# hangxu0304/DeepReduce

Hardware: NVIDIA H100
Metric: ResNet-50 images/sec (whole job, device-timed, max over ranks) (higher is better)
Workload: dtype bf16

## Files before the change

### deepreduce_b200/models/resnet.py

```python
from __future__ import annotations

import torch.nn as nn
import torch.nn.functional as F

from .fused_bn import bn_add_relu, bn_bn_add_relu, bn_relu, bn_relu_maxpool


class _BasicCifar(nn.Module):
    def __init__(self, inp, out, stride):
        super().__init__()
        self.conv1 = nn.Conv2d(inp, out, 3, stride, 1, bias=False)
        self.bn1 = nn.BatchNorm2d(out)
        self.conv2 = nn.Conv2d(out, out, 3, 1, 1, bias=False)
        self.bn2 = nn.BatchNorm2d(out)
        self.pad = None
        if stride != 1 or inp != out:
            self.pad = (out - inp, stride)

    def forward(self, x):
        y = F.relu(self.bn1(self.conv1(x)))
        y = self.bn2(self.conv2(y))
        if self.pad is not None:
            extra, s = self.pad
            x = F.pad(x[:, :, ::s, ::s], (0, 0, 0, 0, extra // 2, extra - extra // 2))
        return F.relu(x + y)


class ResNetCifar(nn.Module):
    def __init__(self, n: int = 3, num_classes: int = 10):
        super().__init__()
        self.conv1 = nn.Conv2d(3, 16, 3, 1, 1, bias=False)
        self.bn1 = nn.BatchNorm2d(16)
        layers, inp = [], 16
        for out, stride in ((16, 1), (32, 2), (64, 2)):
            for i in range(n):
                layers.append(_BasicCifar(inp, out, stride if i == 0 else 1))
                inp = out
        self.layers = nn.Sequential(*layers)
        self.fc = nn.Linear(64, num_classes)

    def forward(self, x):
        x = F.relu(self.bn1(self.conv1(x)))
        x = self.layers(x)
        x = F.adaptive_avg_pool2d(x, 1).flatten(1)
        return self.fc(x)


def resnet20(num_classes: int = 10) -> ResNetCifar:
    return ResNetCifar(3, num_classes)


class _Bottleneck(nn.Module):
    expansion = 4

    def __init__(self, inp, width, stride, downsample):
        super().__init__()
        out = width * self.expansion
        self.conv1 = nn.Conv2d(inp, width, 1, bias=False)
        self.bn1 = nn.BatchNorm2d(width)
        self.conv2 = nn.Conv2d(width, width, 3, stride, 1, bias=False)
        self.bn2 = nn.BatchNorm2d(width)
        self.conv3 = nn.Conv2d(width, out, 1, bias=False)
        self.bn3 = nn.BatchNorm2d(out)
        self.downsample = None
        if downsample:
            self.downsample = nn.Sequential(nn.Conv2d(inp, out, 1, stride, bias=False), nn.BatchNorm2d(out))

    def forward(self, x, skip=None, fork=False):
        skip = x if skip is None else skip
        xd = None if self.downsample is None else self.downsample[0](skip)
        y = bn_relu(self.conv1(x), self.bn1)
        y = bn_relu(self.conv2(y), self.bn2)
        y = self.conv3(y)
        if xd is None:
            return bn_add_relu(y, self.bn3, skip, fork=fork)
        o = bn_bn_add_relu(y, self.bn3, xd, self.downsample[1])
        return (o, None) if fork else o


class ResNet(nn.Module):
    def __init__(self, blocks=(3, 4, 6, 3), num_classes: int = 1000):
        super().__init__()
        self.conv1 = nn.Conv2d(3, 64, 7, 2, 3, bias=False)
        self.bn1 = nn.BatchNorm2d(64)
        self.maxpool = nn.MaxPool2d(3, 2, 1)
        stages, inp = [], 64
        for i, (n, width) in enumerate(zip(blocks, (64, 128, 256, 512))):
            for j in range(n):
                stride = 2 if (j == 0 and i > 0) else 1
                stages.append(_Bottleneck(inp, width, stride, downsample=(j == 0)))
                inp = width * 4
        self.layers = nn.Sequential(*stages)
        self.fc = nn.Linear(inp, num_classes)
        for m in self.modules():
            if isinstance(m, nn.Conv2d):
                nn.init.kaiming_normal_(m.weight, mode="fan_out", nonlinearity="relu")

    def forward(self, x):
        x, skip = bn_relu_maxpool(self.conv1(x), self.bn1, self.maxpool), None
        for blk in self.layers:
            x, skip = blk(x, skip, fork=True)
        x = F.adaptive_avg_pool2d(x, 1).flatten(1)
        return self.fc(x)


def resnet50(num_classes: int = 1000) -> ResNet:
    return ResNet((3, 4, 6, 3), num_classes)
```

### deepreduce_b200/ops/csrc/bn.cu

```cuda
#include <cuda_bf16.h>

#include <algorithm>

#include "common.cuh"
#include "ops.h"

namespace dr {

namespace {

constexpr int kVec = 8;
constexpr int kApplyThreads = 256;
constexpr int kReduceThreads = 128;

struct ChanParams {
  float m[kVec], inv[kVec], w[kVec], b[kVec];
};

__device__ __forceinline__ void load8(const float* __restrict__ p, float* d) {
  const float4 a = __ldg(reinterpret_cast<const float4*>(p));
  const float4 b = __ldg(reinterpret_cast<const float4*>(p) + 1);
  d[0] = a.x; d[1] = a.y; d[2] = a.z; d[3] = a.w;
  d[4] = b.x; d[5] = b.y; d[6] = b.z; d[7] = b.w;
}

__device__ __forceinline__ void load_params(const BnParams& p, int c, ChanParams& o) {
  load8(p.mean + c, o.m);
  load8(p.invstd + c, o.inv);
  load8(p.weight + c, o.w);
  load8(p.bias + c, o.b);
}

__device__ __forceinline__ float bn_elem(float x, float m, float inv, float w, float b) {
  return __fmaf_rn(__fmul_rn(w, __fsub_rn(x, m)), inv, b);
}

__device__ __forceinline__ __nv_bfloat16 relu_bf16(__nv_bfloat16 v) {
  return __bfloat162float(v) <= 0.f ? __float2bfloat16_rn(0.f) : v;
}

__device__ __forceinline__ uint4 add_bf16x8(const uint4& a, const uint4& b) {
  uint4 s;
  const __nv_bfloat16* ha = reinterpret_cast<const __nv_bfloat16*>(&a);
  const __nv_bfloat16* hb = reinterpret_cast<const __nv_bfloat16*>(&b);
  __nv_bfloat16* hs = reinterpret_cast<__nv_bfloat16*>(&s);
#pragma unroll
  for (int i = 0; i < kVec; ++i) hs[i] = __float2bfloat16_rn(__fadd_rn(__bfloat162float(ha[i]), __bfloat162float(hb[i])));
  return s;
}

template <int kMode>
__global__ void __launch_bounds__(kApplyThreads) bn_apply_kernel(const __nv_bfloat16* __restrict__ x, BnParams px,
                                                                 const __nv_bfloat16* __restrict__ z, BnParams pz,
                                                                 __nv_bfloat16* __restrict__ out,
                                                                 uint8_t* __restrict__ mask, int64_t rows, int C) {
  const int groups = C / kVec;
  const int rows_per_cta = blockDim.x / groups;
  const int rsub = threadIdx.x / groups;
  if (rsub >= rows_per_cta) return;
  const int c = (threadIdx.x % groups) * kVec;
  ChanParams a;
  load_params(px, c, a);
  ChanParams d;
  if (kMode == 2) load_params(pz, c, d);
  const int64_t step = (int64_t)gridDim.x * rows_per_cta;
#pragma unroll 2
  for (int64_t r = (int64_t)blockIdx.x * rows_per_cta + rsub; r < rows; r += step) {
    const int64_t off = r * C + c;
    const uint4 vx = *reinterpret_cast<const uint4*>(x + off);
    uint4 vz = make_uint4(0, 0, 0, 0);
    if (kMode != 0) vz = *reinterpret_cast<const uint4*>(z + off);
    const __nv_bfloat16* hx = reinterpret_cast<const __nv_bfloat16*>(&vx);
    const __nv_bfloat16* hz = reinterpret_cast<const __nv_bfloat16*>(&vz);
    uint4 vo;
    __nv_bfloat16* ho = reinterpret_cast<__nv_bfloat16*>(&vo);
    unsigned bits = 0;
#pragma unroll
    for (int i = 0; i < kVec; ++i) {
      __nv_bfloat16 y = __float2bfloat16_rn(bn_elem(__bfloat162float(hx[i]), a.m[i], a.inv[i], a.w[i], a.b[i]));
      if (kMode != 0) {
        const __nv_bfloat16 s = kMode == 1 ? hz[i]
                                           : __float2bfloat16_rn(bn_elem(__bfloat162float(hz[i]), d.m[i], d.inv[i], d.w[i], d.b[i]));
        y = __float2bfloat16_rn(__fadd_rn(__bfloat162float(y), __bfloat162float(s)));
      }
      ho[i] = relu_bf16(y);
      bits |= (__bfloat162float(ho[i]) <= 0.f ? 0u : 1u) << i;
    }
    *reinterpret_cast<uint4*>(out + off) = vo;
    mask[r * groups + c / kVec] = (uint8_t)bits;
  }
}


__global__ void __launch_bounds__(kApplyThreads) bn_apply_pool_kernel(const __nv_bfloat16* __restrict__ x, BnParams px,
                                                                      __nv_bfloat16* __restrict__ out,
                                                                      uint8_t* __restrict__ codes, int64_t orows,
                                                                      PoolGeom pg, int C) {
  const int groups = C / kVec;
  const int rows_per_cta = blockDim.x / groups;
  const int rsub = threadIdx.x / groups;
  if (rsub >= rows_per_cta) return;
  const int c = (threadIdx.x % groups) * kVec;
  ChanParams a;
  load_params(px, c, a);
  const int64_t step = (int64_t)gridDim.x * rows_per_cta;
  for (int64_t r = (int64_t)blockIdx.x * rows_per_cta + rsub; r < orows; r += step) {
    const int ow = (int)(r % pg.Wo);
    const int64_t t = r / pg.Wo;
    const int oh = (int)(t % pg.Ho);
    const int64_t n = t / pg.Ho;
    const int h0 = 2 * oh - 1, w0 = 2 * ow - 1;
    uint4 v[9];
#pragma unroll
    for (int k = 0; k < 9; ++k) {
      const int ih = h0 + k / 3, iw = w0 + k % 3;
      v[k] = ih >= 0 && ih < pg.H && iw >= 0 && iw < pg.W
                 ? *reinterpret_cast<const uint4*>(x + ((n * pg.H + ih) * pg.W + iw) * C + c)
                 : uint4{};
    }
    __nv_bfloat16 best[kVec];
    unsigned slot[kVec];
#pragma unroll
    for (int i = 0; i < kVec; ++i) {
      best[i] = __float2bfloat16_rn(-INFINITY);
      slot[i] = 0;
    }
#pragma unroll
    for (int k = 0; k < 9; ++k) {
      const int ih = h0 + k / 3, iw = w0 + k % 3;
      if (ih < 0 || ih >= pg.H || iw < 0 || iw >= pg.W) continue;
      const __nv_bfloat16* hx = reinterpret_cast<const __nv_bfloat16*>(&v[k]);
#pragma unroll
      for (int i = 0; i < kVec; ++i) {
        const __nv_bfloat16 y = relu_bf16(__float2bfloat16_rn(bn_elem(__bfloat162float(hx[i]), a.m[i], a.inv[i], a.w[i], a.b[i])));
        const float fy = __bfloat162float(y);
        if (fy > __bfloat162float(best[i]) || isnan(fy)) {
          best[i] = y;
          slot[i] = k;
        }
      }
    }
    uint4 vo;
    __nv_bfloat16* ho = reinterpret_cast<__nv_bfloat16*>(&vo);
    uint2 vc;
    uint8_t* hc = reinterpret_cast<uint8_t*>(&vc);
#pragma unroll
    for (int i = 0; i < kVec; ++i) {
      ho[i] = best[i];
      hc[i] = (uint8_t)(slot[i] | (__bfloat162float(best[i]) <= 0.f ? 0u : 0x80u));
    }
    *reinterpret_cast<uint4*>(out + r * C + c) = vo;
    *reinterpret_cast<uint2*>(codes + r * C + c) = vc;
  }
}

struct PoolGather {
  uint4 g[4];
  uint2 code[4];
  int off;
  int nh, nw;
  int sh, sw;
};

__device__ __forceinline__ void pool_gather_codes(PoolGather& q, const uint8_t* __restrict__ codes, const PoolGeom& pg,
                                                  int row, int C, int c, bool valid) {
  const int w = row % pg.W, t = row / pg.W, h = t % pg.H, n = t / pg.H;
  const int ph = h >> 1, pw = w >> 1;
  q.nh = valid ? min((h + 1) / 2 + 1, pg.Ho) - ph : 0;
  q.nw = valid ? min((w + 1) / 2 + 1, pg.Wo) - pw : 0;
  q.sh = h - 2 * ph + 1;
  q.sw = w - 2 * pw + 1;
  q.off = ((n * pg.Ho + ph) * pg.Wo + pw) * C + c;
#pragma unroll
  for (int k = 0; k < 4; ++k) {
    const int a = k >> 1, b = k & 1;
    q.code[k] = a < q.nh && b < q.nw ? *reinterpret_cast<const uint2*>(codes + q.off + (a * pg.Wo + b) * C) : uint2{};
  }
}

template <bool kTwo>
__device__ __forceinline__ void pool_gather_grads(PoolGather& q, const __nv_bfloat16* __restrict__ gp,
                                                  const __nv_bfloat16* __restrict__ gp2, const PoolGeom& pg, int C) {
#pragma unroll
  for (int k = 0; k < 4; ++k) {
    const int a = k >> 1, b = k & 1;
    const bool in = a < q.nh && b < q.nw;
    const int off = q.off + (a * pg.Wo + b) * C;
    q.g[k] = in ? *reinterpret_cast<const uint4*>(gp + off) : uint4{};
    if (kTwo && in) q.g[k] = add_bf16x8(q.g[k], *reinterpret_cast<const uint4*>(gp2 + off));
  }
}

__device__ __forceinline__ void pool_gather_resolve(const PoolGather& q, uint4& g, unsigned& bits) {
  __nv_bfloat16* hg = reinterpret_cast<__nv_bfloat16*>(&g);
  const bool single = q.nh == 1 && q.nw == 1;
  bits = 0;
#pragma unroll
  for (int i = 0; i < kVec; ++i) {
    float s = 0.f;
    __nv_bfloat16 one = __float2bfloat16_rn(0.f);
    unsigned bit = 0;
#pragma unroll
    for (int k = 0; k < 4; ++k) {
      const int a = k >> 1, b = k & 1;
      const unsigned code = (reinterpret_cast<const uint8_t*>(&q.code[k]))[i];
      if (a < q.nh && b < q.nw && (int)(code & 0x7fu) == (q.sh - 2 * a) * 3 + (q.sw - 2 * b)) {
        const __nv_bfloat16 v = (reinterpret_cast<const __nv_bfloat16*>(&q.g[k]))[i];
        s = __fadd_rn(s, __bfloat162float(v));
        one = v;
        bit = code >> 7;
      }
    }
    hg[i] = single ? one : __float2bfloat16_rn(s);
    bits |= bit << i;
  }
}

template <bool kTwo>
__global__ void __launch_bounds__(kApplyThreads) bn_pool_grad_kernel(const __nv_bfloat16* __restrict__ gp,
                                                                     const __nv_bfloat16* __restrict__ gp2,
                                                                     const uint8_t* __restrict__ codes,
                                                                     __nv_bfloat16* __restrict__ g, PoolGeom pg,
                                                                     int64_t rows, int C) {
  const int groups = C / kVec;
  const int rows_per_cta = blockDim.x / groups;
  const int rsub = threadIdx.x / groups;
  if (rsub >= rows_per_cta) return;
  const int c = (threadIdx.x % groups) * kVec;
  const int64_t step = (int64_t)gridDim.x * rows_per_cta;
#pragma unroll 2
  for (int64_t r = (int64_t)blockIdx.x * rows_per_cta + rsub; r < rows; r += step) {
    PoolGather q;
    pool_gather_codes(q, codes, pg, (int)r, C, c, true);
    pool_gather_grads<kTwo>(q, gp, gp2, pg, C);
    uint4 v;
    unsigned bits;
    pool_gather_resolve(q, v, bits);
    __nv_bfloat16* hv = reinterpret_cast<__nv_bfloat16*>(&v);
#pragma unroll
    for (int i = 0; i < kVec; ++i)
      if (!((bits >> i) & 1u)) hv[i] = __float2bfloat16_rn(0.f);
    *reinterpret_cast<uint4*>(g + r * C + c) = v;
  }
}

struct RowTree {
  int block_y, grid_y;
  __host__ __device__ int S() const { return block_y * grid_y; }
  __host__ __device__ int loops(int rows) const { return 1 + (rows - 1) / (S() * kLoads); }
  static constexpr int kLoads = 4;
};

constexpr int kStatsThreads = 256;

__device__ __forceinline__ void welford_update(float x, float inv, float valid, float& mean, float& m2n) {
  const float d0 = __fsub_rn(x, mean);
  mean = __fmaf_rn(d0, inv, mean);
  const float d1 = __fsub_rn(x, mean);
  m2n = __fmaf_rn(__fmul_rn(d0, d1), valid, m2n);
}

template <int kN, bool kFuseNew>
__device__ __forceinline__ void welford_merge(int& n, float* mean, float* m2n, int n_new, const float* mean_new,
                                              const float* m2n_new) {
  const float fn = (float)n, fn_new = (float)n_new;
  const float factor = __frcp_rn((float)max(1, n + n_new));
#pragma unroll
  for (int i = 0; i < kN; ++i) {
    const float d = __fsub_rn(mean[i], mean_new[i]);
    const float s = kFuseNew ? __fmaf_rn(mean_new[i], fn_new, __fmul_rn(mean[i], fn))
                             : __fmaf_rn(mean[i], fn, __fmul_rn(mean_new[i], fn_new));
    mean[i] = __fmul_rn(s, factor);
    const float u = __fmul_rn(__fmul_rn(__fmul_rn(d, d), fn_new), fn);
    m2n[i] = __fadd_rn(m2n[i], __fmaf_rn(u, factor, m2n_new[i]));
  }
  n += n_new;
}

template <int kN>
struct WelfordSlots {
  float* mean; float* m2n; int* count;
  __device__ WelfordSlots(float* sh, int slots)
      : mean(sh), m2n(sh + slots * kN), count(reinterpret_cast<int*>(sh + 2 * slots * kN)) {}
  __device__ void put(int s, int n, const float* m, const float* q) const {
#pragma unroll
    for (int i = 0; i < kN; ++i) { mean[s * kN + i] = m[i]; m2n[s * kN + i] = q[i]; }
    count[s] = n;
  }
  template <bool kFuseNew>
  __device__ void merge_from(int s, int& n, float* m, float* q) const {
    float mn[kN], qn[kN];
#pragma unroll
    for (int i = 0; i < kN; ++i) { mn[i] = mean[s * kN + i]; qn[i] = m2n[s * kN + i]; }
    welford_merge<kN, kFuseNew>(n, m, q, count[s], mn, qn);
  }
  static size_t bytes(int slots) { return (size_t)slots * (2 * kN * sizeof(float) + sizeof(int)); }
};

template <int kN>
__device__ __forceinline__ void welford_tree_over_y(const WelfordSlots<kN>& sl, bool part, int y, int block_y, int base,
                                                    int stride, int& n, float* mean, float* m2n) {
  for (int off = block_y / 2; off > 0; off >>= 1) {
    if (part && y < 2 * off) sl.put(base + y * stride, n, mean, m2n);
    __syncthreads();
    if (part && y < off) sl.template merge_from<false>(base + (y + off) * stride, n, mean, m2n);
    __syncthreads();
  }
}

struct StatsOut {
  float* mean; float* invstd; float* running_mean; float* running_var;
  float* st_mean; float* st_m2n; int* st_count;
  float momentum, bessel, eps;
};

__device__ __forceinline__ void stats_store(const StatsOut& o, int c, int n, float mean, float m2n) {
  const float var = __fdiv_rn(m2n, (float)n);
  const float keep = __fsub_rn(1.f, o.momentum);
  o.mean[c] = mean;
  o.invstd[c] = rsqrtf(__fadd_rn(var, o.eps));
  o.running_mean[c] = __fmaf_rn(mean, o.momentum, __fmul_rn(o.running_mean[c], keep));
  o.running_var[c] = __fmaf_rn(__fmul_rn(var, o.bessel), o.momentum, __fmul_rn(o.running_var[c], keep));
}

__global__ void __launch_bounds__(kStatsThreads) bn_stats_kernel(const __nv_bfloat16* __restrict__ x, StatsOut o,
                                                                 RowTree t, int rows, int C) {
  constexpr int L = RowTree::kLoads;
  constexpr int kAhead = 4;
  extern __shared__ float sh[];
  const int gpc = blockDim.x / (L * t.block_y);
  const int g = threadIdx.x % gpc, j = (threadIdx.x / gpc) % L, y = threadIdx.x / (gpc * L);
  const int group = blockIdx.x * gpc + g;
  const bool live = group * kVec < C;
  const int c = live ? group * kVec : 0;
  const int S = t.S();
  const int n_loops = t.loops(rows);
  const int r0 = blockIdx.y * t.block_y + y + j * S;
  const int rstep = L * S;
  float mean[kVec], m2n[kVec];
#pragma unroll
  for (int i = 0; i < kVec; ++i) mean[i] = m2n[i] = 0.f;
  int n = 0;
  auto load = [&](uint4* b, int i0) {
#pragma unroll
    for (int u = 0; u < kAhead; ++u) {
      const int r = r0 + (i0 + u) * rstep;
      b[u] = live && i0 + u < n_loops && r < rows ? *reinterpret_cast<const uint4*>(x + (size_t)r * C + c) : uint4{};
    }
  };
  uint4 cur[kAhead];
  load(cur, 0);
  for (int i0 = 0; i0 < n_loops; i0 += kAhead) {
    uint4 nxt[kAhead];
    load(nxt, i0 + kAhead);
#pragma unroll
    for (int u = 0; u < kAhead; ++u) {
      const int i = i0 + u;
      if (i >= n_loops) break;
      const bool valid = r0 + i * rstep < rows;
      const float inv = valid ? __frcp_rn((float)(i + 1)) : 0.f;
      const float fv = valid ? 1.f : 0.f;
      n += valid;
      const __nv_bfloat16* hx = reinterpret_cast<const __nv_bfloat16*>(&cur[u]);
#pragma unroll
      for (int k = 0; k < kVec; ++k) welford_update(__bfloat162float(hx[k]), inv, fv, mean[k], m2n[k]);
    }
#pragma unroll
    for (int u = 0; u < kAhead; ++u) cur[u] = nxt[u];
  }
  const WelfordSlots<kVec> sl(sh, blockDim.x);
  sl.put(threadIdx.x, n, mean, m2n);
  __syncthreads();
  if (j == 0) {
#pragma unroll
    for (int a = 1; a < L; ++a) sl.merge_from<true>(threadIdx.x + a * gpc, n, mean, m2n);
  }
  __syncthreads();
  welford_tree_over_y<kVec>(sl, j == 0, y, t.block_y, g, gpc * L, n, mean, m2n);
  if (j != 0 || y != 0 || !live) return;
  if (t.grid_y == 1) {
#pragma unroll
    for (int i = 0; i < kVec; ++i) stats_store(o, c + i, n, mean[i], m2n[i]);
    return;
  }
#pragma unroll
  for (int i = 0; i < kVec; ++i) {
    o.st_mean[(size_t)blockIdx.y * C + c + i] = mean[i];
    o.st_m2n[(size_t)blockIdx.y * C + c + i] = m2n[i];
  }
  if (group == 0) o.st_count[blockIdx.y] = n;
}

__global__ void bn_stats_finalize_kernel(StatsOut o, RowTree t, int C) {
  extern __shared__ float sh[];
  const int cols = blockDim.x / t.block_y;
  const int col = threadIdx.x % cols, y = threadIdx.x / cols;
  const int c = blockIdx.x * cols + col;
  int n = 0;
  float mean = 0.f, m2n = 0.f;
  if (c < C)
    for (int b = y; b < t.grid_y; b += t.block_y) {
      const float mb = o.st_mean[(size_t)b * C + c], qb = o.st_m2n[(size_t)b * C + c];
      welford_merge<1, false>(n, &mean, &m2n, o.st_count[b], &mb, &qb);
    }
  const WelfordSlots<1> sl(sh, blockDim.x);
  welford_tree_over_y<1>(sl, true, y, t.block_y, col, cols, n, &mean, &m2n);
  if (y == 0 && c < C) stats_store(o, c, n, mean, m2n);
}


template <int kN>
__device__ __forceinline__ void tree_over_y(float* v, float* sh, int y, int n, int col, int width) {
  for (int off = n / 2; off > 0; off >>= 1) {
#pragma unroll
    for (int i = 0; i < kN; ++i) sh[y * width + col + i] = v[i];
    __syncthreads();
    if (y < off) {
#pragma unroll
      for (int i = 0; i < kN; ++i) v[i] = __fadd_rn(v[i], sh[(y + off) * width + col + i]);
    }
    __syncthreads();
  }
}

struct BwdOut {
  float* sums;
  float* dw; float* db; float* dwz; float* dbz;
  float* staging;
};

__device__ __forceinline__ void bwd_store(const BwdOut& o, int k, int c, int C, float v, const float* invstd,
                                         const float* invstd_z) {
  o.sums[k * C + c] = v;
  if (k == 0) {
    o.db[c] = v;
    if (o.dbz) o.dbz[c] = v;
  } else if (k == 1) {
    o.dw[c] = __fmul_rn(v, invstd[c]);
  } else {
    o.dwz[c] = __fmul_rn(v, invstd_z[c]);
  }
}

__device__ __forceinline__ float masked(__nv_bfloat16 go, unsigned bit) { return bit ? __bfloat162float(go) : 0.f; }

template <int kMode, bool kTwo>
__global__ void __launch_bounds__(kReduceThreads) bn_bwd_reduce_kernel(const __nv_bfloat16* __restrict__ go,
                                                                       const __nv_bfloat16* __restrict__ go2,
                                                                       const uint8_t* __restrict__ mask,
                                                                       const __nv_bfloat16* __restrict__ x,
                                                                       const float* __restrict__ mean,
                                                                       const float* __restrict__ invstd,
                                                                       const __nv_bfloat16* __restrict__ z,
                                                                       const float* __restrict__ mean_z,
                                                                       const float* __restrict__ invstd_z,
                                                                       __nv_bfloat16* __restrict__ g_out, BwdOut o,
                                                                       RowTree t, int rows, int C) {
  constexpr int kSums = kMode == 2 ? 3 : 2;
  constexpr int L = RowTree::kLoads;
  extern __shared__ float sh[];
  const int gpc = blockDim.x / t.block_y;
  const int tg = threadIdx.x % gpc, y = threadIdx.x / gpc;
  const int group = blockIdx.x * gpc + tg;
  const bool live = group * kVec < C;
  const int c = live ? group * kVec : 0;
  const int S = t.S();
  float m[kVec], mz[kVec];
#pragma unroll
  for (int i = 0; i < kVec; ++i) {
    m[i] = mean[c + i];
    mz[i] = kMode == 2 ? mean_z[c + i] : 0.f;
  }
  float acc[kSums][L][kVec];
#pragma unroll
  for (int k = 0; k < kSums; ++k)
#pragma unroll
    for (int j = 0; j < L; ++j)
#pragma unroll
      for (int i = 0; i < kVec; ++i) acc[k][j][i] = 0.f;
  const int mgroups = C / kVec;
  int r = blockIdx.y * t.block_y + y;
  const int n_loops = t.loops(rows);
  constexpr bool kAhead = !(kTwo && kMode == 2);
  struct Batch {
    uint4 g[L], g2[L], x[L], z[L];
    unsigned m[L];
  };
  auto load = [&](Batch& b, int r0) {
#pragma unroll
    for (int j = 0; j < L; ++j) {
      const int rr = r0 + j * S;
      if (live && rr < rows) {
        const int off = rr * C + c;
        b.g[j] = *reinterpret_cast<const uint4*>(go + off);
        if (kTwo) b.g2[j] = *reinterpret_cast<const uint4*>(go2 + off);
        b.x[j] = *reinterpret_cast<const uint4*>(x + off);
        if (kMode == 2) b.z[j] = *reinterpret_cast<const uint4*>(z + off);
        b.m[j] = kMode == 3 ? 0u : mask[rr * mgroups + group];
      } else {
        b.g[j] = uint4{}; b.g2[j] = uint4{}; b.x[j] = uint4{}; b.z[j] = uint4{}; b.m[j] = 0;
      }
    }
  };
  Batch cur;
  if (kAhead) load(cur, r);
  for (int it = 0; it < n_loops; ++it) {
    if (!kAhead) load(cur, r);
    if (kTwo) {
#pragma unroll
      for (int j = 0; j < L; ++j) cur.g[j] = add_bf16x8(cur.g[j], cur.g2[j]);
    }
    Batch nxt;
    if (kAhead) load(nxt, r + L * S);
    const unsigned* mb = cur.m;
#pragma unroll
    for (int j = 0; j < L; ++j) {
      const __nv_bfloat16* hg = reinterpret_cast<const __nv_bfloat16*>(&cur.g[j]);
      const __nv_bfloat16* hx = reinterpret_cast<const __nv_bfloat16*>(&cur.x[j]);
      const __nv_bfloat16* hz = reinterpret_cast<const __nv_bfloat16*>(&cur.z[j]);
      uint4 vo;
      __nv_bfloat16* ho = reinterpret_cast<__nv_bfloat16*>(&vo);
#pragma unroll
      for (int i = 0; i < kVec; ++i) {
        const unsigned bit = (mb[j] >> i) & 1u;
        const float g = kMode == 3 ? __bfloat162float(hg[i]) : masked(hg[i], bit);
        if (kMode == 1) ho[i] = bit ? hg[i] : __float2bfloat16_rn(0.f);
        acc[0][j][i] = __fadd_rn(acc[0][j][i], g);
        acc[1][j][i] = __fmaf_rn(__fsub_rn(__bfloat162float(hx[i]), m[i]), g, acc[1][j][i]);
        if (kMode == 2) acc[2][j][i] = __fmaf_rn(__fsub_rn(__bfloat162float(hz[i]), mz[i]), g, acc[2][j][i]);
      }
      if (kMode == 1 && live && r + j * S < rows) *reinterpret_cast<uint4*>(g_out + (r + j * S) * C + c) = vo;
    }
    if (kAhead) cur = nxt;
    r += L * S;
  }
#pragma unroll
  for (int k = 0; k < kSums; ++k) {
#pragma unroll
    for (int i = 0; i < kVec; ++i)
#pragma unroll
      for (int j = 1; j < L; ++j) acc[k][0][i] = __fadd_rn(acc[k][0][i], acc[k][j][i]);
    tree_over_y<kVec>(acc[k][0], sh, y, t.block_y, tg * kVec, gpc * kVec);
  }
  if (y != 0 || !live) return;
#pragma unroll
  for (int k = 0; k < kSums; ++k)
#pragma unroll
    for (int i = 0; i < kVec; ++i) {
      if (t.grid_y > 1) o.staging[((size_t)k * t.grid_y + blockIdx.y) * C + c + i] = acc[k][0][i];
      else bwd_store(o, k, c + i, C, acc[k][0][i], invstd, invstd_z);
    }
}

__global__ void bn_bwd_finalize_kernel(BwdOut o, RowTree t, int n_sums, int C, const float* __restrict__ invstd,
                                       const float* __restrict__ invstd_z) {
  extern __shared__ float sh[];
  const int cols = blockDim.x / t.block_y;
  const int col = threadIdx.x % cols, y = threadIdx.x / cols;
  const int c = blockIdx.x * cols + col;
  for (int k = 0; k < n_sums; ++k) {
    float v = 0.f;
    if (c < C)
      for (int b = y; b < t.grid_y; b += t.block_y) v = __fadd_rn(v, o.staging[((size_t)k * t.grid_y + b) * C + c]);
    tree_over_y<1>(&v, sh, y, t.block_y, col, cols);
    if (y == 0 && c < C) bwd_store(o, k, c, C, v, invstd, invstd_z);
  }
}

struct ElemtChan {
  float m[kVec], f1[kVec], f2[kVec], sdy[kVec];
};

__device__ __forceinline__ void elemt_params(const float* mean, const float* invstd, const float* w, const float* sdy,
                                             const float* sxmu, float norm, int c, ElemtChan& p) {
  float inv[kVec], ww[kVec], sx[kVec];
  load8(mean + c, p.m);
  load8(invstd + c, inv);
  load8(w + c, ww);
  load8(sdy + c, p.sdy);
  load8(sxmu + c, sx);
#pragma unroll
  for (int i = 0; i < kVec; ++i) {
    p.f1[i] = __fmul_rn(__fmul_rn(__fmul_rn(inv[i], inv[i]), sx[i]), norm);
    p.f2[i] = __fmul_rn(ww[i], inv[i]);
  }
}

__device__ __forceinline__ __nv_bfloat16 elemt(float g, float x, const ElemtChan& p, int i, float norm) {
  const float a = __fmaf_rn(-p.sdy[i], norm, g);
  return __float2bfloat16_rn(__fmul_rn(__fmaf_rn(-p.f1[i], __fsub_rn(x, p.m[i]), a), p.f2[i]));
}

struct ElemtArgs {
  const float *mean, *invstd, *weight, *sums;
  const float *mean_z, *invstd_z, *weight_z;
};

template <int kMode, bool kTwo>
__global__ void __launch_bounds__(kApplyThreads) bn_bwd_elemt_kernel(const __nv_bfloat16* __restrict__ g_in,
                                                                     const __nv_bfloat16* __restrict__ g2_in,
                                                                     const uint8_t* __restrict__ mask,
                                                                     const __nv_bfloat16* __restrict__ x,
                                                                     const __nv_bfloat16* __restrict__ z, ElemtArgs a,
                                                                     __nv_bfloat16* __restrict__ dx,
                                                                     __nv_bfloat16* __restrict__ dz, float norm,
                                                                     int64_t rows, int C) {
  const int groups = C / kVec;
  const int rows_per_cta = blockDim.x / groups;
  const int rsub = threadIdx.x / groups;
  if (rsub >= rows_per_cta) return;
  const int c = (threadIdx.x % groups) * kVec;
  ElemtChan p;
  elemt_params(a.mean, a.invstd, a.weight, a.sums, a.sums + C, norm, c, p);
  ElemtChan q;
  if (kMode == 2) elemt_params(a.mean_z, a.invstd_z, a.weight_z, a.sums, a.sums + 2 * C, norm, c, q);
  const int64_t step = (int64_t)gridDim.x * rows_per_cta;
#pragma unroll 2
  for (int64_t r = (int64_t)blockIdx.x * rows_per_cta + rsub; r < rows; r += step) {
    const int64_t off = r * C + c;
    uint4 vg = *reinterpret_cast<const uint4*>(g_in + off);
    if (kTwo) vg = add_bf16x8(vg, *reinterpret_cast<const uint4*>(g2_in + off));
    const unsigned mb = kMode == 1 || kMode == 3 ? 0xffu : mask[r * groups + c / kVec];
    const uint4 vx = *reinterpret_cast<const uint4*>(x + off);
    uint4 vz = make_uint4(0, 0, 0, 0);
    if (kMode == 2) vz = *reinterpret_cast<const uint4*>(z + off);
    const __nv_bfloat16* hg = reinterpret_cast<const __nv_bfloat16*>(&vg);
    const __nv_bfloat16* hx = reinterpret_cast<const __nv_bfloat16*>(&vx);
    const __nv_bfloat16* hz = reinterpret_cast<const __nv_bfloat16*>(&vz);
    uint4 vo, vd;
    __nv_bfloat16* ho = reinterpret_cast<__nv_bfloat16*>(&vo);
    __nv_bfloat16* hd = reinterpret_cast<__nv_bfloat16*>(&vd);
#pragma unroll
    for (int i = 0; i < kVec; ++i) {
      const float g = masked(hg[i], (mb >> i) & 1u);
      ho[i] = elemt(g, __bfloat162float(hx[i]), p, i, norm);
      if (kMode == 2) hd[i] = elemt(g, __bfloat162float(hz[i]), q, i, norm);
    }
    *reinterpret_cast<uint4*>(dx + off) = vo;
    if (kMode == 2) *reinterpret_cast<uint4*>(dz + off) = vd;
  }
}

__global__ void bn_update_stats_kernel(const float* __restrict__ mean, float* __restrict__ var_invstd,
                                       float* __restrict__ running_mean, float* __restrict__ running_var, int C,
                                       float momentum, float bessel, float eps) {
  const int c = blockIdx.x * blockDim.x + threadIdx.x;
  if (c >= C) return;
  const float m = mean[c], v = var_invstd[c];
  const float unbiased_var = v * bessel;
  running_mean[c] = m * momentum + (1 - momentum) * running_mean[c];
  running_var[c] = unbiased_var * momentum + (1 - momentum) * running_var[c];
  var_invstd[c] = rsqrtf(v + eps);
}

template <typename K>
cudaError_t rows_grid(K kernel, int64_t rows, int C, int& grid, int& threads) {
  const int groups = C / kVec;
  const int rows_per_cta = groups >= kApplyThreads ? 1 : kApplyThreads / groups;
  threads = groups * rows_per_cta;
  int per_sm = 0;
  cudaError_t e = cudaOccupancyMaxActiveBlocksPerMultiprocessor(&per_sm, kernel, threads, 0);
  if (e != cudaSuccess) return e;
  int64_t g = (rows + rows_per_cta - 1) / rows_per_cta;
  const int64_t cap = (int64_t)(per_sm > 0 ? per_sm : 1) * sm_count();
  grid = (int)(g > cap ? cap : g);
  return cudaSuccess;
}

template <int kMode>
cudaError_t launch_apply(const void* x, const BnParams& px, const void* z, const BnParams& pz, void* out, void* mask,
                         int64_t rows, int C, cudaStream_t st) {
  if (rows == 0) return cudaSuccess;
  int grid = 0, threads = 0;
  cudaError_t e = rows_grid(bn_apply_kernel<kMode>, rows, C, grid, threads);
  if (e != cudaSuccess) return e;
  count_launch();
  bn_apply_kernel<kMode><<<grid, threads, 0, st>>>(reinterpret_cast<const __nv_bfloat16*>(x), px,
                                                   reinterpret_cast<const __nv_bfloat16*>(z), pz,
                                                   reinterpret_cast<__nv_bfloat16*>(out),
                                                   reinterpret_cast<uint8_t*>(mask), rows, C);
  return cudaGetLastError();
}

int last_pow2(unsigned n) {
  n |= n >> 1; n |= n >> 2; n |= n >> 4; n |= n >> 8; n |= n >> 16;
  return std::max<int>(1, (int)(n - (n >> 1)));
}

RowTree row_tree(int rows, int C) {
  const int block_x = std::min(last_pow2((unsigned)C), 32);
  const int block_y = std::min(last_pow2((unsigned)((rows + 15) / 16)), 512 / block_x);
  int grid_y = std::min((rows + block_y * 16 - 1) / (block_y * 16), 128);
  if (grid_y < 8) grid_y = 1;
  return {block_y, grid_y};
}

template <int kMode, bool kTwo>
cudaError_t launch_bwd_reduce(const BnBwd& b, const RowTree& t, const BwdOut& o, int rows, int C, cudaStream_t st) {
  const int groups = C / kVec;
  const int gpc = std::min(groups, std::max(1, kReduceThreads / t.block_y));
  const dim3 grid((groups + gpc - 1) / gpc, t.grid_y);
  const int threads = gpc * t.block_y;
  count_launch();
  bn_bwd_reduce_kernel<kMode, kTwo><<<grid, threads, threads * kVec * sizeof(float), st>>>(
      reinterpret_cast<const __nv_bfloat16*>(b.go), reinterpret_cast<const __nv_bfloat16*>(b.go2), b.mask,
      reinterpret_cast<const __nv_bfloat16*>(b.x), b.px.mean, b.px.invstd, reinterpret_cast<const __nv_bfloat16*>(b.z),
      b.pz.mean, b.pz.invstd, reinterpret_cast<__nv_bfloat16*>(b.g), o, t, rows, C);
  return cudaGetLastError();
}

template <int kMode, bool kTwo>
cudaError_t launch_bwd_elemt(const BnBwd& b, const ElemtArgs& a, int64_t rows, int C, cudaStream_t st) {
  int grid = 0, threads = 0;
  cudaError_t e = rows_grid(bn_bwd_elemt_kernel<kMode, kTwo>, rows, C, grid, threads);
  if (e != cudaSuccess) return e;
  const float norm = (float)(1.0 / (double)rows);
  count_launch();
  bn_bwd_elemt_kernel<kMode, kTwo><<<grid, threads, 0, st>>>(
      reinterpret_cast<const __nv_bfloat16*>(kMode == 1 || kMode == 3 ? b.g : b.go),
      reinterpret_cast<const __nv_bfloat16*>(b.go2), b.mask, reinterpret_cast<const __nv_bfloat16*>(b.x),
      reinterpret_cast<const __nv_bfloat16*>(b.z), a, reinterpret_cast<__nv_bfloat16*>(b.dx),
      reinterpret_cast<__nv_bfloat16*>(b.dz), norm, rows, C);
  return cudaGetLastError();
}

template <int kMode, bool kTwo>
cudaError_t launch_backward(const BnBwd& b, int64_t rows64, int C, cudaStream_t st) {
  const int rows = (int)rows64;
  const RowTree t = row_tree(rows, C);
  const BwdOut o{b.sums, b.dw, b.db, b.dwz, b.dbz, b.staging};
  cudaError_t e;
  if (kMode == 3) {
    int grid = 0, threads = 0;
    e = rows_grid(bn_pool_grad_kernel<kTwo>, rows64, C, grid, threads);
    if (e != cudaSuccess) return e;
    count_launch();
    bn_pool_grad_kernel<kTwo><<<grid, threads, 0, st>>>(reinterpret_cast<const __nv_bfloat16*>(b.go),
                                                        reinterpret_cast<const __nv_bfloat16*>(b.go2), b.mask,
                                                        reinterpret_cast<__nv_bfloat16*>(b.g), b.pool, rows64, C);
    e = cudaGetLastError();
    if (e != cudaSuccess) return e;
  }
  BnBwd bb = b;
  if (kMode == 3) bb.go = b.g;
  e = launch_bwd_reduce<kMode, kTwo && kMode != 3>(bb, t, o, rows, C, st);
  if (e != cudaSuccess) return e;
  if (t.grid_y > 1) {
    const int cols = std::max(1, 512 / t.block_y);
    const int threads = cols * t.block_y;
    count_launch();
    bn_bwd_finalize_kernel<<<(C + cols - 1) / cols, threads, threads * sizeof(float), st>>>(
        o, t, kMode == 2 ? 3 : 2, C, b.px.invstd, b.pz.invstd);
    e = cudaGetLastError();
    if (e != cudaSuccess) return e;
  }
  const ElemtArgs a{b.px.mean, b.px.invstd, b.px.weight, b.sums, b.pz.mean, b.pz.invstd, b.pz.weight};
  return launch_bwd_elemt<kMode, kTwo && kMode == 2>(b, a, rows64, C, st);
}

cudaError_t launch_stats(const BnStats& s, int rows, int C, cudaStream_t st) {
  const RowTree t = row_tree(rows, C);
  const int grid_y = t.grid_y;
  const StatsOut o{s.mean, s.invstd, s.running_mean, s.running_var,
                   s.staging, s.staging + (size_t)grid_y * C, reinterpret_cast<int*>(s.staging + 2 * (size_t)grid_y * C),
                   s.momentum, s.bessel, s.eps};
  const int groups = C / kVec;
  const int gpc = std::min(groups, std::max(1, kStatsThreads / (RowTree::kLoads * t.block_y)));
  const int threads = gpc * RowTree::kLoads * t.block_y;
  count_launch();
  bn_stats_kernel<<<dim3((groups + gpc - 1) / gpc, grid_y), threads, WelfordSlots<kVec>::bytes(threads), st>>>(
      reinterpret_cast<const __nv_bfloat16*>(s.x), o, t, rows, C);
  cudaError_t e = cudaGetLastError();
  if (e != cudaSuccess || grid_y == 1) return e;
  const int cols = std::max(1, 512 / t.block_y);
  const int fthreads = cols * t.block_y;
  count_launch();
  bn_stats_finalize_kernel<<<(C + cols - 1) / cols, fthreads, WelfordSlots<1>::bytes(fthreads), st>>>(o, t, C);
  return cudaGetLastError();
}

}

void bn_row_tree(int64_t rows, int C, int* block_y, int* grid_y) {
  const RowTree t = row_tree((int)rows, C);
  *block_y = t.block_y;
  *grid_y = t.grid_y;
}

cudaError_t launch_bn_backward(int mode, const BnBwd& b, int64_t rows, int C, cudaStream_t st) {
  if (rows == 0) return cudaSuccess;
  const bool two = b.go2 != nullptr;
  switch (mode) {
    case 0: return two ? cudaErrorInvalidValue : launch_backward<0, false>(b, rows, C, st);
    case 1: return two ? launch_backward<1, true>(b, rows, C, st) : launch_backward<1, false>(b, rows, C, st);
    case 2: return two ? launch_backward<2, true>(b, rows, C, st) : launch_backward<2, false>(b, rows, C, st);
    case 3: return two ? launch_backward<3, true>(b, rows, C, st) : launch_backward<3, false>(b, rows, C, st);
    default: return cudaErrorInvalidValue;
  }
}

cudaError_t launch_bn_stats(const BnStats& s, int64_t rows, int C, cudaStream_t st) {
  if (rows == 0) return cudaSuccess;
  return launch_stats(s, (int)rows, C, st);
}

cudaError_t launch_bn_update_stats(const float* mean, float* var_invstd, float* running_mean, float* running_var, int C,
                                   float momentum, float bessel, float eps, cudaStream_t st) {
  count_launch();
  bn_update_stats_kernel<<<(C + 255) / 256, 256, 0, st>>>(mean, var_invstd, running_mean, running_var, C, momentum,
                                                          bessel, eps);
  return cudaGetLastError();
}

cudaError_t launch_bn_apply(int mode, const void* x, const BnParams& px, const void* z, const BnParams& pz, void* out,
                            void* mask, int64_t rows, int C, cudaStream_t st) {
  switch (mode) {
    case 0: return launch_apply<0>(x, px, z, pz, out, mask, rows, C, st);
    case 1: return launch_apply<1>(x, px, z, pz, out, mask, rows, C, st);
    case 2: return launch_apply<2>(x, px, z, pz, out, mask, rows, C, st);
    default: return cudaErrorInvalidValue;
  }
}

cudaError_t launch_bn_apply_pool(const void* x, const BnParams& px, void* out, void* codes, int N, const PoolGeom& pg,
                                 int C, cudaStream_t st) {
  const int64_t orows = (int64_t)N * pg.Ho * pg.Wo;
  if (orows == 0) return cudaSuccess;
  int grid = 0, threads = 0;
  cudaError_t e = rows_grid(bn_apply_pool_kernel, orows, C, grid, threads);
  if (e != cudaSuccess) return e;
  count_launch();
  bn_apply_pool_kernel<<<grid, threads, 0, st>>>(reinterpret_cast<const __nv_bfloat16*>(x), px,
                                                 reinterpret_cast<__nv_bfloat16*>(out),
                                                 reinterpret_cast<uint8_t*>(codes), orows, pg, C);
  return cudaGetLastError();
}

}
```

Before: 6168.

## Tile stem BN+ReLU+maxpool kernels through cp.async shared-memory row rings

The fused stem BN-ReLU-maxpool forward kernel and its backward gradient scatter kernel are rewritten to tile spatial bands and column chunks. Input rows are staged in a shared-memory ring with cp.async pipelining, so each input pixel is normalised once and reused across overlapping 3x3 windows instead of being reloaded up to nine times. The max and slot search, and the backward resolve, now use packed bf16x2 masks and byte tricks rather than scalar loops. The model also forks the skip from the stem output, and the kernels gain dynamic shared-memory setup and more complex indexing.

```diff
diff --git a/deepreduce_b200/models/resnet.py b/deepreduce_b200/models/resnet.py
--- a/deepreduce_b200/models/resnet.py
+++ b/deepreduce_b200/models/resnet.py
@@ -97,7 +97,7 @@
                 nn.init.kaiming_normal_(m.weight, mode="fan_out", nonlinearity="relu")
 
     def forward(self, x):
-        x, skip = bn_relu_maxpool(self.conv1(x), self.bn1, self.maxpool), None
+        x, skip = bn_relu_maxpool(self.conv1(x), self.bn1, self.maxpool, fork=True)
         for blk in self.layers:
             x, skip = blk(x, skip, fork=True)
         x = F.adaptive_avg_pool2d(x, 1).flatten(1)
diff --git a/deepreduce_b200/ops/csrc/bn.cu b/deepreduce_b200/ops/csrc/bn.cu
--- a/deepreduce_b200/ops/csrc/bn.cu
+++ b/deepreduce_b200/ops/csrc/bn.cu
@@ -91,156 +91,228 @@
   }
 }
 
-
-__global__ void __launch_bounds__(kApplyThreads) bn_apply_pool_kernel(const __nv_bfloat16* __restrict__ x, BnParams px,
-                                                                      __nv_bfloat16* __restrict__ out,
-                                                                      uint8_t* __restrict__ codes, int64_t orows,
-                                                                      PoolGeom pg, int C) {
-  const int groups = C / kVec;
-  const int rows_per_cta = blockDim.x / groups;
-  const int rsub = threadIdx.x / groups;
-  if (rsub >= rows_per_cta) return;
-  const int c = (threadIdx.x % groups) * kVec;
+constexpr int kPoolThreads = 256;
+constexpr int kPoolBand = 8;
+constexpr int kPoolMaxG = 8;
+constexpr int kFwdDepth = 2, kFwdRing = 2 * kFwdDepth + 3;
+constexpr int kGradDepth = 4, kGradRing = kGradDepth + 2;
+constexpr int kFwdRowEntries = 2 * kPoolThreads + kPoolMaxG;
+constexpr size_t kFwdSmem = (size_t)kFwdRing * kFwdRowEntries * sizeof(uint4);
+
+struct PoolTiles {
+  int gshift;
+  int ncol;
+  int nbands;
+};
+
+__device__ __forceinline__ uint4 relu_bn8(const uint4 vx, const ChanParams& a) {
+  uint4 vy;
+  const __nv_bfloat16* hx = reinterpret_cast<const __nv_bfloat16*>(&vx);
+  __nv_bfloat16* hy = reinterpret_cast<__nv_bfloat16*>(&vy);
+#pragma unroll
+  for (int i = 0; i < kVec; ++i)
+    hy[i] = relu_bf16(__float2bfloat16_rn(bn_elem(__bfloat162float(hx[i]), a.m[i], a.inv[i], a.w[i], a.b[i])));
+  return vy;
+}
+
+__global__ void __launch_bounds__(kPoolThreads) bn_apply_pool_kernel(const __nv_bfloat16* __restrict__ x, BnParams px,
+                                                                     __nv_bfloat16* __restrict__ out,
+                                                                     uint8_t* __restrict__ codes, PoolGeom pg,
+                                                                     PoolTiles pt, int C) {
+  extern __shared__ uint4 ring[];
+  auto row_of = [&](int r) { return ring + (r + kFwdRing) % kFwdRing * kFwdRowEntries; };
+  const int G = 1 << pt.gshift, TW = kPoolThreads >> pt.gshift, S = 2 * TW + 1;
+  const int gi = threadIdx.x & (G - 1), j = threadIdx.x >> pt.gshift;
+  const int c = (blockIdx.y * G + gi) * kVec;
+  const int chunk = blockIdx.x % pt.ncol, band = blockIdx.x / pt.ncol % pt.nbands;
+  const int n = blockIdx.x / pt.ncol / pt.nbands;
+  const int ow0 = chunk * TW, iw0 = 2 * ow0 - 1;
+  const int oh0 = band * kPoolBand, oh1 = min(oh0 + kPoolBand, pg.Ho);
+  const int rlo = 2 * oh0 - 1;
+  const __nv_bfloat16* xn = x + (size_t)n * pg.H * pg.W * C + c;
   ChanParams a;
   load_params(px, c, a);
-  const int64_t step = (int64_t)gridDim.x * rows_per_cta;
-  for (int64_t r = (int64_t)blockIdx.x * rows_per_cta + rsub; r < orows; r += step) {
-    const int ow = (int)(r % pg.Wo);
-    const int64_t t = r / pg.Wo;
-    const int oh = (int)(t % pg.Ho);
-    const int64_t n = t / pg.Ho;
-    const int h0 = 2 * oh - 1, w0 = 2 * ow - 1;
-    uint4 v[9];
-#pragma unroll
-    for (int k = 0; k < 9; ++k) {
-      const int ih = h0 + k / 3, iw = w0 + k % 3;
-      v[k] = ih >= 0 && ih < pg.H && iw >= 0 && iw < pg.W
-                 ? *reinterpret_cast<const uint4*>(x + ((n * pg.H + ih) * pg.W + iw) * C + c)
-                 : uint4{};
-    }
-    __nv_bfloat16 best[kVec];
-    unsigned slot[kVec];
-#pragma unroll
-    for (int i = 0; i < kVec; ++i) {
-      best[i] = __float2bfloat16_rn(-INFINITY);
-      slot[i] = 0;
-    }
-#pragma unroll
-    for (int k = 0; k < 9; ++k) {
-      const int ih = h0 + k / 3, iw = w0 + k % 3;
-      if (ih < 0 || ih >= pg.H || iw < 0 || iw >= pg.W) continue;
-      const __nv_bfloat16* hx = reinterpret_cast<const __nv_bfloat16*>(&v[k]);
-#pragma unroll
-      for (int i = 0; i < kVec; ++i) {
-        const __nv_bfloat16 y = relu_bf16(__float2bfloat16_rn(bn_elem(__bfloat162float(hx[i]), a.m[i], a.inv[i], a.w[i], a.b[i])));
-        const float fy = __bfloat162float(y);
-        if (fy > __bfloat162float(best[i]) || isnan(fy)) {
-          best[i] = y;
-          slot[i] = k;
+
+  auto fetch = [&](int r0) {
+#pragma unroll
+    for (int k = 0; k < 2; ++k) {
+      const int r = r0 + k;
+#pragma unroll
+      for (int i = 0; i < 3; ++i) {
+        const int s = j + i * TW, iw = iw0 + s;
+        if (r >= rlo && r >= 0 && r < pg.H && s < S && iw >= 0 && iw < pg.W)
+          cp_async_16(row_of(r) + s * G + gi, xn + (r * pg.W + iw) * C);
+      }
+    }
+    cp_async_commit();
+  };
+  auto finish = [&](int r0) {
+    const uint4 ninf = make_uint4(0xff80ff80u, 0xff80ff80u, 0xff80ff80u, 0xff80ff80u);
+#pragma unroll
+    for (int k = 0; k < 2; ++k) {
+      const int r = r0 + k;
+      if (r < rlo) continue;
+      uint4* row = row_of(r);
+#pragma unroll
+      for (int i = 0; i < 3; ++i) {
+        const int s = j + i * TW, iw = iw0 + s;
+        if (s >= S) continue;
+        row[s * G + gi] = r >= 0 && r < pg.H && iw >= 0 && iw < pg.W ? relu_bn8(row[s * G + gi], a) : ninf;
+      }
+    }
+  };
+
+  const int ow = ow0 + j;
+  for (int d = 0; d < kFwdDepth; ++d) fetch(2 * (oh0 - 1 + d));
+  for (int oh = oh0 - 1; oh < oh1; ++oh) {
+    cp_async_wait<kFwdDepth - 1>();
+    finish(2 * oh);
+    __syncthreads();
+    if (oh + kFwdDepth < oh1) fetch(2 * (oh + kFwdDepth));
+    else cp_async_commit();
+    if (oh < oh0 || ow >= pg.Wo) continue;
+    unsigned best[kVec / 2], slot[kVec / 2];
+#pragma unroll
+    for (int p = 0; p < kVec / 2; ++p) {
+      best[p] = 0xff80ff80u;
+      slot[p] = 0;
+    }
+#pragma unroll
+    for (int kh = 0; kh < 3; ++kh) {
+      const uint4* row = row_of(2 * oh - 1 + kh);
+#pragma unroll
+      for (int kw = 0; kw < 3; ++kw) {
+        const uint4 vy = row[(2 * j + kw) * G + gi];
+        const unsigned* v = reinterpret_cast<const unsigned*>(&vy);
+#pragma unroll
+        for (int p = 0; p < kVec / 2; ++p) {
+          const __nv_bfloat162 v2 = *reinterpret_cast<const __nv_bfloat162*>(&v[p]);
+          const unsigned m = __hgt2_mask(v2, *reinterpret_cast<const __nv_bfloat162*>(&best[p])) | __hneu2_mask(v2, v2);
+          best[p] = (v[p] & m) | (best[p] & ~m);
+          slot[p] = ((unsigned)(kh * 3 + kw) * 0x10001u & m) | (slot[p] & ~m);
         }
       }
     }
-    uint4 vo;
-    __nv_bfloat16* ho = reinterpret_cast<__nv_bfloat16*>(&vo);
+    uint4 vo = make_uint4(best[0], best[1], best[2], best[3]);
+    const __nv_bfloat16* ho = reinterpret_cast<const __nv_bfloat16*>(&vo);
     uint2 vc;
     uint8_t* hc = reinterpret_cast<uint8_t*>(&vc);
 #pragma unroll
-    for (int i = 0; i < kVec; ++i) {
-      ho[i] = best[i];
-      hc[i] = (uint8_t)(slot[i] | (__bfloat162float(best[i]) <= 0.f ? 0u : 0x80u));
-    }
-    *reinterpret_cast<uint4*>(out + r * C + c) = vo;
-    *reinterpret_cast<uint2*>(codes + r * C + c) = vc;
+    for (int i = 0; i < kVec; ++i)
+      hc[i] = (uint8_t)((slot[i / 2] >> 16 * (i % 2) & 0xfu) | (__bfloat162float(ho[i]) <= 0.f ? 0u : 0x80u));
+    const size_t off = (((size_t)n * pg.Ho + oh) * pg.Wo + ow) * C + c;
+    *reinterpret_cast<uint4*>(out + off) = vo;
+    *reinterpret_cast<uint2*>(codes + off) = vc;
   }
 }
 
 struct PoolGather {
   uint4 g[4];
   uint2 code[4];
-  int off;
   int nh, nw;
   int sh, sw;
 };
 
-__device__ __forceinline__ void pool_gather_codes(PoolGather& q, const uint8_t* __restrict__ codes, const PoolGeom& pg,
-                                                  int row, int C, int c, bool valid) {
-  const int w = row % pg.W, t = row / pg.W, h = t % pg.H, n = t / pg.H;
-  const int ph = h >> 1, pw = w >> 1;
-  q.nh = valid ? min((h + 1) / 2 + 1, pg.Ho) - ph : 0;
-  q.nw = valid ? min((w + 1) / 2 + 1, pg.Wo) - pw : 0;
-  q.sh = h - 2 * ph + 1;
-  q.sw = w - 2 * pw + 1;
-  q.off = ((n * pg.Ho + ph) * pg.Wo + pw) * C + c;
-#pragma unroll
-  for (int k = 0; k < 4; ++k) {
+template <int kA>
+__device__ __forceinline__ uint4 pool_gather_resolve(const PoolGather& q) {
+  unsigned gm[2 * kA][4], won[2] = {0, 0};
+#pragma unroll
+  for (int k = 0; k < 2 * kA; ++k) {
     const int a = k >> 1, b = k & 1;
-    q.code[k] = a < q.nh && b < q.nw ? *reinterpret_cast<const uint2*>(codes + q.off + (a * pg.Wo + b) * C) : uint2{};
-  }
+    const unsigned slot = (unsigned)((q.sh - 2 * a) * 3 + (q.sw - 2 * b)) * 0x01010101u;
+    const unsigned* gw = reinterpret_cast<const unsigned*>(&q.g[k]);
+#pragma unroll
+    for (int h = 0; h < 2; ++h) {
+      const unsigned code = h ? q.code[k].y : q.code[k].x;
+      const unsigned x = (code ^ slot) & 0x7f7f7f7fu;
+      unsigned t = ~((x + 0x7f7f7f7fu) | x) & 0x80808080u;
+      if (!(a < q.nh && b < q.nw)) t = 0;
+      won[h] |= t & code;
+      const unsigned m8 = (t >> 7) * 0xffu;
+      gm[k][2 * h] = gw[2 * h] & __byte_perm(m8, 0, 0x1100);
+      gm[k][2 * h + 1] = gw[2 * h + 1] & __byte_perm(m8, 0, 0x3322);
+    }
+  }
+  const bool single = q.nh == 1 && q.nw == 1;
+  uint4 g;
+  unsigned* ow = reinterpret_cast<unsigned*>(&g);
+#pragma unroll
+  for (int w = 0; w < 4; ++w) {
+    float lo = 0.f, hi = 0.f;
+#pragma unroll
+    for (int k = 0; k < 2 * kA; ++k) {
+      lo = __fadd_rn(lo, __uint_as_float(gm[k][w] << 16));
+      hi = __fadd_rn(hi, __uint_as_float(gm[k][w] & 0xffff0000u));
+    }
+    const unsigned sum = (unsigned)__bfloat16_as_ushort(__float2bfloat16_rn(lo)) |
+                         (unsigned)__bfloat16_as_ushort(__float2bfloat16_rn(hi)) << 16;
+    const unsigned m8 = (won[w / 2] >> 7 & 0x01010101u) * 0xffu;
+    ow[w] = (single ? gm[0][w] : sum) &
+            __byte_perm(m8, 0, w % 2 ? 0x3322 : 0x1100);
+  }
+  return g;
 }
 
 template <bool kTwo>
-__device__ __forceinline__ void pool_gather_grads(PoolGather& q, const __nv_bfloat16* __restrict__ gp,
-                                                  const __nv_bfloat16* __restrict__ gp2, const PoolGeom& pg, int C) {
-#pragma unroll
-  for (int k = 0; k < 4; ++k) {
-    const int a = k >> 1, b = k & 1;
-    const bool in = a < q.nh && b < q.nw;
-    const int off = q.off + (a * pg.Wo + b) * C;
-    q.g[k] = in ? *reinterpret_cast<const uint4*>(gp + off) : uint4{};
-    if (kTwo && in) q.g[k] = add_bf16x8(q.g[k], *reinterpret_cast<const uint4*>(gp2 + off));
-  }
-}
-
-__device__ __forceinline__ void pool_gather_resolve(const PoolGather& q, uint4& g, unsigned& bits) {
-  __nv_bfloat16* hg = reinterpret_cast<__nv_bfloat16*>(&g);
-  const bool single = q.nh == 1 && q.nw == 1;
-  bits = 0;
-#pragma unroll
-  for (int i = 0; i < kVec; ++i) {
-    float s = 0.f;
-    __nv_bfloat16 one = __float2bfloat16_rn(0.f);
-    unsigned bit = 0;
-#pragma unroll
-    for (int k = 0; k < 4; ++k) {
-      const int a = k >> 1, b = k & 1;
-      const unsigned code = (reinterpret_cast<const uint8_t*>(&q.code[k]))[i];
-      if (a < q.nh && b < q.nw && (int)(code & 0x7fu) == (q.sh - 2 * a) * 3 + (q.sw - 2 * b)) {
-        const __nv_bfloat16 v = (reinterpret_cast<const __nv_bfloat16*>(&q.g[k]))[i];
-        s = __fadd_rn(s, __bfloat162float(v));
-        one = v;
-        bit = code >> 7;
+__global__ void __launch_bounds__(kPoolThreads, kTwo ? 5 : 4) bn_pool_grad_kernel(const __nv_bfloat16* __restrict__ gp,
+                                                                    const __nv_bfloat16* __restrict__ gp2,
+                                                                    const uint8_t* __restrict__ codes,
+                                                                    __nv_bfloat16* __restrict__ g, PoolGeom pg,
+                                                                    PoolTiles pt, int C) {
+  constexpr int kRow = kPoolThreads / 2 + kPoolMaxG;
+  __shared__ uint4 sg[kGradRing][kRow];
+  __shared__ uint4 sg2[kTwo ? kGradRing : 1][kRow];
+  __shared__ uint2 sc[kGradRing][kRow];
+  const int G = 1 << pt.gshift, TWp = (kPoolThreads / 2) >> pt.gshift;
+  const int gi = threadIdx.x & (G - 1), wl = threadIdx.x >> pt.gshift;
+  const int c = (blockIdx.y * G + gi) * kVec;
+  const int chunk = blockIdx.x % pt.ncol, band = blockIdx.x / pt.ncol % pt.nbands;
+  const int n = blockIdx.x / pt.ncol / pt.nbands;
+  const int pw0 = chunk * TWp, w = 2 * pw0 + wl;
+  const int oh0 = band * kPoolBand, oh1 = min(oh0 + kPoolBand, pg.Ho);
+  const size_t pbase = (size_t)n * pg.Ho * pg.Wo * C + c;
+  const bool stager = wl <= TWp && pw0 + wl < pg.Wo;
+  const int se = wl * G + gi;
+
+  auto fetch = [&](int p) {
+    if (stager && p < pg.Ho) {
+      const size_t off = pbase + (size_t)(p * pg.Wo + pw0 + wl) * C;
+      cp_async_16(&sg[p % kGradRing][se], gp + off);
+      if (kTwo) cp_async_16(&sg2[p % kGradRing][se], gp2 + off);
+      cp_async_8(&sc[p % kGradRing][se], codes + off);
+    }
+    cp_async_commit();
+  };
+
+  const int nw = min((w + 1) / 2 + 1, pg.Wo) - (w >> 1);
+  for (int d = 0; d < kGradDepth; ++d) fetch(oh0 + d <= oh1 ? oh0 + d : pg.Ho);
+  for (int m = oh0 - 1; m < oh1; ++m) {
+    cp_async_wait<kGradDepth - 1>();
+    const int s1 = (m + 1) % kGradRing;
+    if (kTwo && stager && m + 1 < pg.Ho) sg[s1][se] = add_bf16x8(sg[s1][se], sg2[s1][se]);
+    __syncthreads();
+    fetch(m + 1 + kGradDepth <= oh1 ? m + 1 + kGradDepth : pg.Ho);
+    if (m < oh0 || w >= pg.W) continue;
+#pragma unroll
+    for (int k2 = 0; k2 < 2; ++k2) {
+      const int h = 2 * m + k2;
+      if (h >= pg.H) break;
+      PoolGather q;
+      q.nh = k2 ? min(m + 2, pg.Ho) - m : 1;
+      q.nw = nw;
+      q.sh = k2 + 1;
+      q.sw = (w & 1) + 1;
+#pragma unroll
+      for (int k = 0; k < 4; ++k) {
+        const int a = k >> 1, b = k & 1;
+        const int e = ((wl >> 1) + b) * G + gi;
+        const bool in = a < q.nh && b < q.nw;
+        q.g[k] = in ? sg[(m + a) % kGradRing][e] : uint4{};
+        q.code[k] = in ? sc[(m + a) % kGradRing][e] : uint2{};
       }
-    }
-    hg[i] = single ? one : __float2bfloat16_rn(s);
-    bits |= bit << i;
-  }
-}
-
-template <bool kTwo>
-__global__ void __launch_bounds__(kApplyThreads) bn_pool_grad_kernel(const __nv_bfloat16* __restrict__ gp,
-                                                                     const __nv_bfloat16* __restrict__ gp2,
-                                                                     const uint8_t* __restrict__ codes,
-                                                                     __nv_bfloat16* __restrict__ g, PoolGeom pg,
-                                                                     int64_t rows, int C) {
-  const int groups = C / kVec;
-  const int rows_per_cta = blockDim.x / groups;
-  const int rsub = threadIdx.x / groups;
-  if (rsub >= rows_per_cta) return;
-  const int c = (threadIdx.x % groups) * kVec;
-  const int64_t step = (int64_t)gridDim.x * rows_per_cta;
-#pragma unroll 2
-  for (int64_t r = (int64_t)blockIdx.x * rows_per_cta + rsub; r < rows; r += step) {
-    PoolGather q;
-    pool_gather_codes(q, codes, pg, (int)r, C, c, true);
-    pool_gather_grads<kTwo>(q, gp, gp2, pg, C);
-    uint4 v;
-    unsigned bits;
-    pool_gather_resolve(q, v, bits);
-    __nv_bfloat16* hv = reinterpret_cast<__nv_bfloat16*>(&v);
-#pragma unroll
-    for (int i = 0; i < kVec; ++i)
-      if (!((bits >> i) & 1u)) hv[i] = __float2bfloat16_rn(0.f);
-    *reinterpret_cast<uint4*>(g + r * C + c) = v;
+      *reinterpret_cast<uint4*>(g + (((size_t)n * pg.H + h) * pg.W + w) * C + c) =
+          k2 ? pool_gather_resolve<2>(q) : pool_gather_resolve<1>(q);
+    }
   }
 }
 
@@ -667,6 +739,16 @@
   return cudaSuccess;
 }
 
+int pool_gshift(int C) {
+  int gs = 3;
+  while ((C / kVec) % (1 << gs)) --gs;
+  return gs;
+}
+
+dim3 pool_grid(int N, const PoolTiles& pt, int C) {
+  return dim3((unsigned)N * pt.nbands * pt.ncol, (C / kVec) >> pt.gshift);
+}
+
 template <int kMode>
 cudaError_t launch_apply(const void* x, const BnParams& px, const void* z, const BnParams& pz, void* out, void* mask,
                          int64_t rows, int C, cudaStream_t st) {
@@ -731,13 +813,14 @@
   const BwdOut o{b.sums, b.dw, b.db, b.dwz, b.dbz, b.staging};
   cudaError_t e;
   if (kMode == 3) {
-    int grid = 0, threads = 0;
-    e = rows_grid(bn_pool_grad_kernel<kTwo>, rows64, C, grid, threads);
-    if (e != cudaSuccess) return e;
+    const int N = (int)(rows64 / ((int64_t)b.pool.H * b.pool.W));
+    const int gs = pool_gshift(C);
+    const PoolTiles pt{gs, (b.pool.Wo + ((kPoolThreads / 2) >> gs) - 1) / ((kPoolThreads / 2) >> gs),
+                       (b.pool.Ho + kPoolBand - 1) / kPoolBand};
     count_launch();
-    bn_pool_grad_kernel<kTwo><<<grid, threads, 0, st>>>(reinterpret_cast<const __nv_bfloat16*>(b.go),
-                                                        reinterpret_cast<const __nv_bfloat16*>(b.go2), b.mask,
-                                                        reinterpret_cast<__nv_bfloat16*>(b.g), b.pool, rows64, C);
+    bn_pool_grad_kernel<kTwo><<<pool_grid(N, pt, C), kPoolThreads, 0, st>>>(
+        reinterpret_cast<const __nv_bfloat16*>(b.go), reinterpret_cast<const __nv_bfloat16*>(b.go2), b.mask,
+        reinterpret_cast<__nv_bfloat16*>(b.g), b.pool, pt, C);
     e = cudaGetLastError();
     if (e != cudaSuccess) return e;
   }
@@ -824,15 +907,15 @@
 
 cudaError_t launch_bn_apply_pool(const void* x, const BnParams& px, void* out, void* codes, int N, const PoolGeom& pg,
                                  int C, cudaStream_t st) {
-  const int64_t orows = (int64_t)N * pg.Ho * pg.Wo;
-  if (orows == 0) return cudaSuccess;
-  int grid = 0, threads = 0;
-  cudaError_t e = rows_grid(bn_apply_pool_kernel, orows, C, grid, threads);
+  if ((int64_t)N * pg.Ho * pg.Wo == 0) return cudaSuccess;
+  const int gs = pool_gshift(C);
+  const PoolTiles pt{gs, (pg.Wo + (kPoolThreads >> gs) - 1) / (kPoolThreads >> gs), (pg.Ho + kPoolBand - 1) / kPoolBand};
+  cudaError_t e = cudaFuncSetAttribute(bn_apply_pool_kernel, cudaFuncAttributeMaxDynamicSharedMemorySize, (int)kFwdSmem);
   if (e != cudaSuccess) return e;
   count_launch();
-  bn_apply_pool_kernel<<<grid, threads, 0, st>>>(reinterpret_cast<const __nv_bfloat16*>(x), px,
-                                                 reinterpret_cast<__nv_bfloat16*>(out),
-                                                 reinterpret_cast<uint8_t*>(codes), orows, pg, C);
+  bn_apply_pool_kernel<<<pool_grid(N, pt, C), kPoolThreads, kFwdSmem, st>>>(reinterpret_cast<const __nv_bfloat16*>(x), px,
+                                                                     reinterpret_cast<__nv_bfloat16*>(out),
+                                                                     reinterpret_cast<uint8_t*>(codes), pg, pt, C);
   return cudaGetLastError();
 }
 
```

Measured after the change: 6250 (median of 6 runs). +1.3%, better.
